# yangsenwxy/VSR

Measured on AMD Instinct MI355X. Metric: voxels/sec fwd+bwd, 4× SR on 16×128×128 cine volumes, 1/2/4/8 MI355X, higher is better.
Workload: dtype bf16

## Files before the change

### vsr_amd/csrc/conv_wgrad_row.hip

```cpp
#include <algorithm>
#include "conv_common.h"

namespace {
using namespace vsrk_conv;

constexpr int RW_NW = 8;
constexpr int RW_KC = 4;
constexpr int RW_SEG = 32 * RW_KC;
constexpr int RW_XV = RW_SEG + 8;
constexpr int RW_XP = RW_XV / 8;
constexpr int RW_YP = RW_SEG / 8;
constexpr int RW_NP = RW_XP + RW_YP;
constexpr int RW_NQ = (RW_NP + RW_NW - 1) / RW_NW;
constexpr int RW_XSLOT = RW_XP * 1024;
constexpr int RW_YSLOT = RW_YP * 1024;
constexpr int RW_NXS = 4, RW_NYS = 2;
constexpr int RW_YBASE = RW_NXS * RW_XSLOT;
constexpr int RW_LDS = RW_YBASE + RW_NYS * RW_YSLOT;
constexpr int RW_COW = 64;
constexpr int RW_SLAB = 9 * RW_COW * 64 + RW_COW;
constexpr uint32_t RW_OOB = 0x80000000u;

#ifndef RW_ABL
#define RW_ABL 0
#endif

__host__ __device__ constexpr int rw_swz(int j) { return 2 * ((j >> 1) & 1) + 4 * ((j >> 3) & 1); }

typedef __amdgpu_buffer_rsrc_t RwRsrc;
__device__ __forceinline__ RwRsrc rw_rsrc(const void* base) {
  const uint64_t b = (uint64_t)base;
  const uint64_t u = ((uint64_t)(uint32_t)__builtin_amdgcn_readfirstlane((int)(uint32_t)(b >> 32)) << 32) |
                     (uint32_t)__builtin_amdgcn_readfirstlane((int)(uint32_t)b);
  return __builtin_amdgcn_make_buffer_rsrc((void*)u, 0, 0x7FFFFFF0, 0x00020000);
}
typedef uint32_t rw_u32x4 __attribute__((ext_vector_type(4)));
__device__ __forceinline__ void rw_st16(uint32_t addr, uint4 v) {
  *(__attribute__((address_space(3))) rw_u32x4*)(size_t)addr = __builtin_bit_cast(rw_u32x4, v);
}

typedef float f32x4_t __attribute__((ext_vector_type(4)));
template <typename H> struct V8R;
template <> struct V8R<bf16> { typedef bf16x8 type; };
template <> struct V8R<f16> { typedef f16x8 type; };
__device__ __forceinline__ f32x4_t rw_mfma(bf16x8 a, bf16x8 b, f32x4_t c) {
  return __builtin_amdgcn_mfma_f32_16x16x32_bf16(a, b, c, 0, 0, 0);
}
__device__ __forceinline__ f32x4_t rw_mfma(f16x8 a, f16x8 b, f32x4_t c) {
  return __builtin_amdgcn_mfma_f32_16x16x32_f16(a, b, c, 0, 0, 0);
}
__device__ __forceinline__ uint4 rw_frag(uint32_t p0, uint32_t p1) {
  const v4i16 a = __builtin_amdgcn_ds_read_tr16_b64_v4i16((lds_v4i16*)(size_t)p0);
  const v4i16 b = __builtin_amdgcn_ds_read_tr16_b64_v4i16((lds_v4i16*)(size_t)p1);
  return __builtin_bit_cast(uint4, __builtin_shufflevector(a, b, 0, 1, 2, 3, 4, 5, 6, 7));
}

constexpr int RW_MAXB = 16;

struct RowArgs {
  const char* x;
  const char* dy;
  int xoff[RW_MAXB], yoff[RW_MAXB];
  uint16_t tapm[RW_MAXB];
  int tapm_x;
  float* ws;
  int64_t xsn, xsd, xsh, xsw, ysn, ysd, ysh, ysw;
  int xd, H, W;
  int bands, band_h, nseg, ncot, ncic, nsplit;
  int want_bias;
  int prio;
};

template <typename H, bool SPM>
__global__ __launch_bounds__(RW_NW * 64, 1) void wgrad_row_kernel(RowArgs a) {
  using V8 = typename V8R<H>::type;
  extern __shared__ __attribute__((aligned(16))) char lds[];
  const int lane = threadIdx.x & 63;
  const int wave = __builtin_amdgcn_readfirstlane(threadIdx.x >> 6);
  const int coh = wave & 1, cib = wave >> 1;

  const int ncombo = a.ncot * a.ncic;
  const int L = xcd_remap(blockIdx.x, a.nsplit * ncombo);
  const int split = L / ncombo;
  const int combo = L - split * ncombo;
  const int cot = combo % a.ncot, cic = combo / a.ncot;
  const int seg = split % a.nseg;
  const int t0 = split / a.nseg;
  const int band = t0 % a.bands, img = t0 / a.bands;
  const int nb = img / a.xd, dd = img - nb * a.xd;
  const int h0 = band * a.band_h;
  const int nst = min(a.H, h0 + a.band_h) - h0;
  const int w0 = seg * RW_SEG;
  const unsigned tapm = SPM ? (unsigned)a.tapm[a.tapm_x ? cic : cot] : 0x1ffu;
  const char* xim = a.x + 2 * (nb * a.xsn + dd * a.xsd + a.xoff[cic]);
  const char* yim = a.dy + 2 * (nb * a.ysn + dd * a.ysd + a.yoff[cot]);

  static_assert(RW_XP == 2 * RW_NW + 1 && RW_YP == 2 * RW_NW, "piece roles");
  uint32_t goff[RW_NQ], loff[RW_NQ];
#pragma unroll
  for (int q = 0; q < RW_NQ; ++q) {
    const bool isx = q != 2 && q != 3;
    const int j = q == 4 ? 2 * RW_NW : wave + RW_NW * (q & 1);
    if (isx) {
      const int v = 8 * j + (lane >> 3);
      const int col = w0 - 1 + v;
      const bool ok = v < RW_SEG + 2 && col >= 0 && col < a.W;
      goff[q] = ok ? (uint32_t)(2 * (col * (int)a.xsw + 8 * (lane & 7))) : RW_OOB;
      loff[q] = (uint32_t)(j * 1024 + (lane >> 3) * 128 + 16 * ((lane & 7) ^ rw_swz(v)));
    } else {
      const int v = 8 * j + (lane >> 3);
      const int col = w0 + v;
      goff[q] = col < a.W ? (uint32_t)(2 * (col * (int)a.ysw + 8 * (lane & 7))) : RW_OOB;
      loff[q] = (uint32_t)(j * 1024 + (lane >> 3) * 128 + 16 * ((lane & 7) ^ rw_swz(v)));
    }
  }
  const uint32_t lbase = lds_addr(lds);
  auto load_set = [&](int t, uint4 (&r)[RW_NQ]) __attribute__((always_inline)) {
    const int xr = h0 - 1 + t;
    const bool xok = xr >= 0 && xr < a.H;
    const int yr = t - 2;
    const bool yok = yr >= 0 && yr < nst;
    const RwRsrc rx = rw_rsrc(xim + 2 * (int64_t)(xok ? xr : 0) * a.xsh);
    const RwRsrc ry = rw_rsrc(yim + 2 * (int64_t)(h0 + (yok ? yr : 0)) * a.ysh);
#pragma unroll
    for (int q = 0; q < RW_NQ; ++q) {
      const bool isx = q != 2 && q != 3;
      if (q == 4 && wave != 0) break;
      r[q] = __builtin_bit_cast(uint4, __builtin_amdgcn_raw_buffer_load_b128(
                                           isx ? rx : ry, (int)((isx ? xok : yok) ? goff[q] : RW_OOB), 0, 0));
    }
  };
  auto store_set = [&](int t, const uint4 (&r)[RW_NQ]) __attribute__((always_inline)) {
    const uint32_t xs = lbase + (uint32_t)(t % RW_NXS) * RW_XSLOT;
    const int yr = t - 2;
    const uint32_t ys = lbase + RW_YBASE + (uint32_t)((yr < 0 ? 0 : yr) % RW_NYS) * RW_YSLOT;
#pragma unroll
    for (int q = 0; q < RW_NQ; ++q) {
      const bool isx = q != 2 && q != 3;
      if (q == 4 && wave != 0) break;
      if (isx) rw_st16(xs + loff[q], r[q]);
      else if (yr >= 0) rw_st16(ys + loff[q], r[q]);
    }
  };

  const int g = lane >> 4, qq = (lane >> 2) & 3, pp = lane & 3;
  uint32_t xo[3][2];
#pragma unroll
  for (int kw = 0; kw < 3; ++kw)
#pragma unroll
    for (int h = 0; h < 2; ++h) {
      const int v = kw + 8 * g + qq + 4 * h;
      xo[kw][h] = (uint32_t)(v * 128 + 16 * ((2 * cib + (pp >> 1)) ^ rw_swz(v)) + 8 * (pp & 1));
    }
  uint32_t yo[2][2];
#pragma unroll
  for (int b = 0; b < 2; ++b)
#pragma unroll
    for (int h = 0; h < 2; ++h) {
      const int v = 8 * g + qq + 4 * h;
      yo[b][h] = (uint32_t)(v * 128 + 16 * ((2 * (2 * coh + b) + (pp >> 1)) ^ rw_swz(v)) + 8 * (pp & 1));
    }

  f32x4_t acc[3][3][2];
#pragma unroll
  for (int i = 0; i < 18; ++i) acc[i / 6][(i / 2) % 3][i % 2] = f32x4_t{0.f, 0.f, 0.f, 0.f};
  f32x4_t bacc[2] = {f32x4_t{0.f, 0.f, 0.f, 0.f}, f32x4_t{0.f, 0.f, 0.f, 0.f}};
  uint4 ones;
  {
    const H one = from_f32<H>(1.f);
    const uint16_t u = __builtin_bit_cast(uint16_t, one);
    const uint32_t w2 = (uint32_t)u | ((uint32_t)u << 16);
    ones = make_uint4(w2, w2, w2, w2);
  }

  const int last = nst + 1;
  uint4 stg[RW_NQ], stg2[RW_NQ];
  load_set(0, stg);
  if (1 <= last) load_set(1, stg2);
  store_set(0, stg);
  if (1 <= last) store_set(1, stg2);
  if (2 <= last) {
    load_set(2, stg);
    store_set(2, stg);
  }
  __syncthreads();
  if (3 <= last) load_set(3, stg);
  __builtin_amdgcn_sched_barrier(0);

  for (int s = 0; s < nst; ++s) {
    uint32_t xa[3][3][2], ya[2][2];
#pragma unroll
    for (int kh = 0; kh < 3; ++kh) {
      const uint32_t xrow = lbase + (uint32_t)((s + kh) % RW_NXS) * RW_XSLOT;
#pragma unroll
      for (int kw = 0; kw < 3; ++kw)
#pragma unroll
        for (int h = 0; h < 2; ++h) {
          xa[kh][kw][h] = xrow + xo[kw][h];
          asm volatile("" : "+v"(xa[kh][kw][h]));
        }
    }
    {
      const uint32_t yr = lbase + RW_YBASE + (uint32_t)(s % RW_NYS) * RW_YSLOT;
#pragma unroll
      for (int b = 0; b < 2; ++b)
#pragma unroll
        for (int h = 0; h < 2; ++h) {
          ya[b][h] = yr + yo[b][h];
          asm volatile("" : "+v"(ya[b][h]));
        }
    }
    uint4 xf[2][3], yf[2][2];
    auto load_group = [&](int G) __attribute__((always_inline)) {
      const int kc = G / 3, kh = G % 3;
      if (kh == 0) {
#pragma unroll
        for (int b = 0; b < 2; ++b) yf[kc & 1][b] = rw_frag(ya[b][0] + kc * 4096, ya[b][1] + kc * 4096);
      }
#pragma unroll
      for (int kw = 0; kw < 3; ++kw) xf[G & 1][kw] = rw_frag(xa[kh][kw][0] + kc * 4096, xa[kh][kw][1] + kc * 4096);
    };
    load_group(0);
#pragma unroll
    for (int G = 0; G < 3 * RW_KC; ++G) {
      if (G + 1 < 3 * RW_KC) load_group(G + 1);
      __builtin_amdgcn_sched_barrier(0);
      if (a.prio) __builtin_amdgcn_s_setprio(1);
      const int kc = G / 3, kh = G % 3;
#pragma unroll
      for (int kw = 0; kw < 3; ++kw) {
        if (SPM && !((tapm >> (kh * 3 + kw)) & 1)) continue;
#pragma unroll
        for (int b = 0; b < 2; ++b)
          if (RW_ABL & 2) acc[kh][kw][b][0] += __builtin_bit_cast(float, yf[kc & 1][b].x ^ xf[G & 1][kw].y);
          else acc[kh][kw][b] = rw_mfma(__builtin_bit_cast(V8, yf[kc & 1][b]), __builtin_bit_cast(V8, xf[G & 1][kw]),
                                   acc[kh][kw][b]);
      }
      if (kh == 1 && kc == cib) {
#pragma unroll
        for (int b = 0; b < 2; ++b)
          bacc[b] = rw_mfma(__builtin_bit_cast(V8, yf[kc & 1][b]), __builtin_bit_cast(V8, ones), bacc[b]);
      }
      if (a.prio) __builtin_amdgcn_s_setprio(0);
      __builtin_amdgcn_sched_barrier(0);
    }
    if (!(RW_ABL & 1)) {
      if (s + 3 <= last) store_set(s + 3, stg);
      asm volatile("s_waitcnt lgkmcnt(0)\n\ts_barrier" ::: "memory");
      if (s + 4 <= last) load_set(s + 4, stg);
    }
    __builtin_amdgcn_sched_barrier(0);
  }

  float* out = a.ws + ((int64_t)split * ncombo + combo) * RW_SLAB;
  const int l15 = lane & 15, lg = lane >> 4;
#pragma unroll
  for (int t9 = 0; t9 < 9; ++t9)
#pragma unroll
    for (int b = 0; b < 2; ++b)
#pragma unroll
      for (int i = 0; i < 4; ++i) {
        const int co = 32 * coh + 16 * b + 4 * lg + i, ci = 16 * cib + l15;
        out[(t9 * RW_COW + co) * 64 + ci] = ((tapm >> t9) & 1) ? acc[t9 / 3][t9 % 3][b][i] : 0.f;
      }
  if (a.want_bias && cic == 0) {
    float* part = reinterpret_cast<float*>(lds);
    __syncthreads();
    if (l15 == 0) {
#pragma unroll
      for (int b = 0; b < 2; ++b)
#pragma unroll
        for (int i = 0; i < 4; ++i) part[cib * 64 + 32 * coh + 16 * b + 4 * lg + i] = bacc[b][i];
    }
    __syncthreads();
    if (threadIdx.x < RW_COW) {
      const int c = threadIdx.x;
      out[9 * RW_COW * 64 + c] = ((part[c] + part[64 + c]) + part[128 + c]) + part[192 + c];
    }
  }
}

const int g_wrow_bands = std::max(0, vsrk_env_int("VSRK_WGRAD_ROW_BANDS", 0));
const int g_wrow_prio = vsrk_env_int("VSRK_WGRAD_ROW_PRIO", 0) == 1;

}

bool vsrk_wgrad_row_plan(const vsrk_conv_desc* d, const vsrk_tensor5* x, const vsrk_tensor5* dy, VsrkRowPlan* p) {
  const int mode = vsrk_path_mode(VSRK_PATH_WGRAD_ROW);
  if (mode == 0) return false;
  if (!vsrk_is16(x->dtype) || dy->dtype != x->dtype) return false;
  if (d->kd != 1 || d->kh != 3 || d->kw != 3 || d->pd != 0 || d->ph != 1 || d->pw != 1) return false;
  if (d->prologue != VSRK_PRO_NONE) return false;
  if (x->c % 64 || dy->c % 64 || (x->shuffle > 1 && dy->shuffle > 1)) return false;
  if (d->subpixel && (x->shuffle > 1 || dy->shuffle > 1) && mode != 2) return false;
  if (x->c / 64 > RW_MAXB || dy->c / 64 > RW_MAXB) return false;
  for (const vsrk_tensor5* t : {x, dy}) {
    if (t->shuffle <= 1) continue;
    const int r = t->shuffle, cph = t->c / (r * r);
    if (cph * r * r != t->c || cph % 64) return false;
  }
  if (x->n != dy->n || x->d != dy->d || x->h != dy->h || x->w != dy->w) return false;
  if (!chunk_ok(x, 2) || !chunk_ok(dy, 2)) return false;
  for (const vsrk_tensor5* t : {x, dy}) {
    const int64_t r = t->shuffle > 1 ? t->shuffle : 1;
    if (t->sn < 0 || t->sd < 0 || t->sh < 0 || t->sw < 0 ||
        (int64_t)(RW_XV + 2) * r * t->sw + (r - 1) * t->sh + t->c >= (1ll << 29))
      return false;
  }
  const int64_t images = (int64_t)x->n * x->d;
  if (images <= 0 || x->h <= 0 || x->w <= 0) return false;
  const int nseg = ceil_div(x->w, RW_SEG);
  const int ncot = dy->c / RW_COW, ncic = x->c / 64;
  const int64_t per_band = images * nseg * ncot * ncic;
  int64_t want = std::max<int64_t>(1, vsrk_num_cus());
  if (vsrk_g_grid_cap > 0) want = std::min<int64_t>(want, vsrk_g_grid_cap);
  int bands = (int)std::max<int64_t>(1, std::min<int64_t>((want + per_band / 2) / per_band, ceil_div(x->h, 8)));
  if (g_wrow_bands > 0) bands = std::min(g_wrow_bands, x->h);
  if (vsrk_g_grid_cap > 0) bands = std::max(1, std::min(bands, x->h));
  p->band_h = ceil_div(x->h, bands);
  p->bands = ceil_div(x->h, p->band_h);
  p->nseg = nseg;
  p->ncot = ncot;
  p->ncic = ncic;
  const int64_t ns = images * p->bands * nseg;
  if (ns * ncot * ncic >= (1ll << 30)) return false;
  p->nsplit = (int)ns;
  p->cot_w = RW_COW;
  p->slab = RW_SLAB;
  p->ws_bytes = (size_t)ns * ncot * ncic * RW_SLAB * sizeof(float);
  return true;
}

int vsrk_conv_wgrad_row(const vsrk_conv_desc* d, const vsrk_tensor5* x, const vsrk_tensor5* dy, int want_bias,
                        float* ws, size_t ws_bytes, VsrkRowPlan* plan, hipStream_t s) {
  VsrkRowPlan p;
  if (!vsrk_wgrad_row_plan(d, x, dy, &p)) return 0;
  if (ws_bytes < p.ws_bytes) return 0;
  RowArgs a;
  a.x = (const char*)x->ptr;
  a.dy = (const char*)dy->ptr;
  a.ws = ws;
  auto blocks = [](const vsrk_tensor5* t, int64_t& sh, int64_t& sw, int* off) {
    const int r = t->shuffle > 1 ? t->shuffle : 1;
    sh = (int64_t)r * t->sh;
    sw = (int64_t)r * t->sw;
    const int cph = t->c / (r * r);
    for (int b = 0; b < t->c / 64; ++b) {
      const int c = 64 * b, sub = c / cph, cc = c - sub * cph;
      off[b] = (int)((sub / r) * t->sh + (sub % r) * t->sw + cc);
    }
  };
  a.xsn = x->sn; a.xsd = x->sd;
  a.ysn = dy->sn; a.ysd = dy->sd;
  blocks(x, a.xsh, a.xsw, a.xoff);
  blocks(dy, a.ysh, a.ysw, a.yoff);
  const vsrk_tensor5* spt = x->shuffle > 1 ? x : (dy->shuffle > 1 ? dy : nullptr);
  const bool spm = d->subpixel && spt;
  a.tapm_x = spt == x;
  if (spm) {
    const int r = spt->shuffle, cph = spt->c / (r * r);
    const int32_t code = d->subpixel & ~(1 << 25);
    for (int b = 0; b < spt->c / 64; ++b) a.tapm[b] = (uint16_t)subpixel_tapmask(code, r, 64 * b / cph);
  }
  a.xd = x->d;
  a.H = x->h;
  a.W = x->w;
  a.bands = p.bands;
  a.band_h = p.band_h;
  a.nseg = p.nseg;
  a.ncot = p.ncot;
  a.ncic = p.ncic;
  a.nsplit = p.nsplit;
  a.want_bias = want_bias;
  a.prio = g_wrow_prio;
  const int grid = p.nsplit * p.ncot * p.ncic;
  vsrk_dispatch16(x->dtype, [&](auto tag) {
    using H = decltype(tag);
    auto kern = spm ? wgrad_row_kernel<H, true> : wgrad_row_kernel<H, false>;
    (void)hipFuncSetAttribute((const void*)kern, hipFuncAttributeMaxDynamicSharedMemorySize, RW_LDS);
    kern<<<grid, RW_NW * 64, RW_LDS, s>>>(a);
    return 0;
  });
  *plan = p;
  return 1;
}
```

Before: 65.30 million.

## Repartition wgrad-row waves across K-chunk halves with LDS cross-wave reduction

Changes the work split in the row weight-gradient kernel. Each wave now owns one 16-wide input-channel block and all 64 output channels, and the two wave groups split the 4 K-chunks two each, instead of splitting output channels in halves. Each x fragment then feeds 4 MFMAs instead of 2, which cuts the LDS read traffic per MFMA. The cost is that the two K halves must be summed through LDS in an epilogue, and accumulator registers double to 36 f32x4. The main loop is also unrolled by the ring depth so slot offsets become immediates, and the unused priority knob is removed.

```diff
diff --git a/vsr_amd/csrc/conv_wgrad_row.hip b/vsr_amd/csrc/conv_wgrad_row.hip
--- a/vsr_amd/csrc/conv_wgrad_row.hip
+++ b/vsr_amd/csrc/conv_wgrad_row.hip
@@ -68,7 +68,6 @@
   int xd, H, W;
   int bands, band_h, nseg, ncot, ncic, nsplit;
   int want_bias;
-  int prio;
 };
 
 template <typename H, bool SPM>
@@ -77,7 +76,7 @@
   extern __shared__ __attribute__((aligned(16))) char lds[];
   const int lane = threadIdx.x & 63;
   const int wave = __builtin_amdgcn_readfirstlane(threadIdx.x >> 6);
-  const int coh = wave & 1, cib = wave >> 1;
+  const int cib = wave & 3, kh2 = wave >> 2;
 
   const int ncombo = a.ncot * a.ncic;
   const int L = xcd_remap(blockIdx.x, a.nsplit * ncombo);
@@ -144,26 +143,45 @@
   };
 
   const int g = lane >> 4, qq = (lane >> 2) & 3, pp = lane & 3;
+  const uint32_t kbase = lbase + (uint32_t)kh2 * (2 * 4096);
   uint32_t xo[3][2];
 #pragma unroll
   for (int kw = 0; kw < 3; ++kw)
 #pragma unroll
     for (int h = 0; h < 2; ++h) {
       const int v = kw + 8 * g + qq + 4 * h;
-      xo[kw][h] = (uint32_t)(v * 128 + 16 * ((2 * cib + (pp >> 1)) ^ rw_swz(v)) + 8 * (pp & 1));
-    }
-  uint32_t yo[2][2];
-#pragma unroll
-  for (int b = 0; b < 2; ++b)
+      xo[kw][h] = kbase + (uint32_t)(v * 128 + 16 * ((2 * cib + (pp >> 1)) ^ rw_swz(v)) + 8 * (pp & 1));
+      asm volatile("" : "+v"(xo[kw][h]));
+    }
+  uint32_t yo[4][2];
+#pragma unroll
+  for (int b = 0; b < 4; ++b)
 #pragma unroll
     for (int h = 0; h < 2; ++h) {
       const int v = 8 * g + qq + 4 * h;
-      yo[b][h] = (uint32_t)(v * 128 + 16 * ((2 * (2 * coh + b) + (pp >> 1)) ^ rw_swz(v)) + 8 * (pp & 1));
-    }
-
-  f32x4_t acc[3][3][2];
-#pragma unroll
-  for (int i = 0; i < 18; ++i) acc[i / 6][(i / 2) % 3][i % 2] = f32x4_t{0.f, 0.f, 0.f, 0.f};
+      yo[b][h] = kbase + RW_YBASE + (uint32_t)(v * 128 + 16 * ((2 * b + (pp >> 1)) ^ rw_swz(v)) + 8 * (pp & 1));
+      asm volatile("" : "+v"(yo[b][h]));
+    }
+  static_assert((RW_NXS - 1) * RW_XSLOT + 4096 < 65536 && (RW_NYS - 1) * RW_YSLOT + 4096 < 65536, "ds offsets");
+
+  const int last = nst + 1;
+  uint4 stg[RW_NQ];
+  {
+    uint4 stg1[RW_NQ], stg2[RW_NQ];
+    load_set(0, stg);
+    load_set(1, stg1);
+    load_set(2, stg2);
+    store_set(0, stg);
+    store_set(1, stg1);
+    store_set(2, stg2);
+  }
+  __syncthreads();
+  if (3 <= last) load_set(3, stg);
+  __builtin_amdgcn_sched_barrier(0);
+
+  f32x4_t acc[3][3][4];
+#pragma unroll
+  for (int i = 0; i < 36; ++i) acc[i / 12][(i / 4) % 3][i % 4] = f32x4_t{0.f, 0.f, 0.f, 0.f};
   f32x4_t bacc[2] = {f32x4_t{0.f, 0.f, 0.f, 0.f}, f32x4_t{0.f, 0.f, 0.f, 0.f}};
   uint4 ones;
   {
@@ -173,115 +191,103 @@
     ones = make_uint4(w2, w2, w2, w2);
   }
 
-  const int last = nst + 1;
-  uint4 stg[RW_NQ], stg2[RW_NQ];
-  load_set(0, stg);
-  if (1 <= last) load_set(1, stg2);
-  store_set(0, stg);
-  if (1 <= last) store_set(1, stg2);
-  if (2 <= last) {
-    load_set(2, stg);
-    store_set(2, stg);
-  }
-  __syncthreads();
-  if (3 <= last) load_set(3, stg);
-  __builtin_amdgcn_sched_barrier(0);
-
-  for (int s = 0; s < nst; ++s) {
-    uint32_t xa[3][3][2], ya[2][2];
-#pragma unroll
-    for (int kh = 0; kh < 3; ++kh) {
-      const uint32_t xrow = lbase + (uint32_t)((s + kh) % RW_NXS) * RW_XSLOT;
-#pragma unroll
-      for (int kw = 0; kw < 3; ++kw)
-#pragma unroll
-        for (int h = 0; h < 2; ++h) {
-          xa[kh][kw][h] = xrow + xo[kw][h];
-          asm volatile("" : "+v"(xa[kh][kw][h]));
+  for (int s4 = 0; s4 < nst; s4 += RW_NXS) {
+#pragma unroll
+    for (int u = 0; u < RW_NXS; ++u) {
+      const int s = s4 + u;
+      if (s >= nst) break;
+      uint4 xf[2][3], yf[4];
+      auto load_x = [&](int G) __attribute__((always_inline)) {
+        const int imm = ((u + G % 3) % RW_NXS) * RW_XSLOT + (G / 3) * 4096;
+#pragma unroll
+        for (int kw = 0; kw < 3; ++kw) xf[G & 1][kw] = rw_frag(xo[kw][0] + imm, xo[kw][1] + imm);
+      };
+      auto load_y = [&](int kc, int b) __attribute__((always_inline)) {
+        const int imm = (u % RW_NYS) * RW_YSLOT + kc * 4096;
+        yf[b] = rw_frag(yo[b][0] + imm, yo[b][1] + imm);
+      };
+#pragma unroll
+      for (int b = 0; b < 4; ++b) load_y(0, b);
+      load_x(0);
+#pragma unroll
+      for (int G = 0; G < 6; ++G) {
+        if (G + 1 < 6) load_x(G + 1);
+        __builtin_amdgcn_sched_barrier(0);
+        const int kc = G / 3, kh = G % 3;
+#pragma unroll
+        for (int b = 0; b < 4; ++b) {
+#pragma unroll
+          for (int kw = 0; kw < 3; ++kw) {
+            if (SPM && !((tapm >> (kh * 3 + kw)) & 1)) continue;
+            if (RW_ABL & 2) acc[kh][kw][b][0] += __builtin_bit_cast(float, yf[b].x ^ xf[G & 1][kw].y);
+            else acc[kh][kw][b] = rw_mfma(__builtin_bit_cast(V8, yf[b]), __builtin_bit_cast(V8, xf[G & 1][kw]),
+                                     acc[kh][kw][b]);
+          }
+          if (kh == 1 && b == cib)
+            bacc[kc] = rw_mfma(__builtin_bit_cast(V8, yf[b]), __builtin_bit_cast(V8, ones), bacc[kc]);
+          if (G == 2) {
+            __builtin_amdgcn_sched_barrier(0);
+            load_y(1, b);
+            __builtin_amdgcn_sched_barrier(0);
+          }
         }
-    }
-    {
-      const uint32_t yr = lbase + RW_YBASE + (uint32_t)(s % RW_NYS) * RW_YSLOT;
-#pragma unroll
-      for (int b = 0; b < 2; ++b)
-#pragma unroll
-        for (int h = 0; h < 2; ++h) {
-          ya[b][h] = yr + yo[b][h];
-          asm volatile("" : "+v"(ya[b][h]));
-        }
-    }
-    uint4 xf[2][3], yf[2][2];
-    auto load_group = [&](int G) __attribute__((always_inline)) {
-      const int kc = G / 3, kh = G % 3;
-      if (kh == 0) {
-#pragma unroll
-        for (int b = 0; b < 2; ++b) yf[kc & 1][b] = rw_frag(ya[b][0] + kc * 4096, ya[b][1] + kc * 4096);
+        __builtin_amdgcn_sched_barrier(0);
       }
-#pragma unroll
-      for (int kw = 0; kw < 3; ++kw) xf[G & 1][kw] = rw_frag(xa[kh][kw][0] + kc * 4096, xa[kh][kw][1] + kc * 4096);
-    };
-    load_group(0);
-#pragma unroll
-    for (int G = 0; G < 3 * RW_KC; ++G) {
-      if (G + 1 < 3 * RW_KC) load_group(G + 1);
+      if (!(RW_ABL & 1)) {
+        if (s + 3 <= last) store_set(s + 3, stg);
+        asm volatile("s_waitcnt lgkmcnt(0)\n\ts_barrier" ::: "memory");
+        if (s + 4 <= last) load_set(s + 4, stg);
+      }
       __builtin_amdgcn_sched_barrier(0);
-      if (a.prio) __builtin_amdgcn_s_setprio(1);
-      const int kc = G / 3, kh = G % 3;
-#pragma unroll
-      for (int kw = 0; kw < 3; ++kw) {
-        if (SPM && !((tapm >> (kh * 3 + kw)) & 1)) continue;
-#pragma unroll
-        for (int b = 0; b < 2; ++b)
-          if (RW_ABL & 2) acc[kh][kw][b][0] += __builtin_bit_cast(float, yf[kc & 1][b].x ^ xf[G & 1][kw].y);
-          else acc[kh][kw][b] = rw_mfma(__builtin_bit_cast(V8, yf[kc & 1][b]), __builtin_bit_cast(V8, xf[G & 1][kw]),
-                                   acc[kh][kw][b]);
-      }
-      if (kh == 1 && kc == cib) {
-#pragma unroll
-        for (int b = 0; b < 2; ++b)
-          bacc[b] = rw_mfma(__builtin_bit_cast(V8, yf[kc & 1][b]), __builtin_bit_cast(V8, ones), bacc[b]);
-      }
-      if (a.prio) __builtin_amdgcn_s_setprio(0);
-      __builtin_amdgcn_sched_barrier(0);
-    }
-    if (!(RW_ABL & 1)) {
-      if (s + 3 <= last) store_set(s + 3, stg);
-      asm volatile("s_waitcnt lgkmcnt(0)\n\ts_barrier" ::: "memory");
-      if (s + 4 <= last) load_set(s + 4, stg);
-    }
-    __builtin_amdgcn_sched_barrier(0);
+    }
   }
 
   float* out = a.ws + ((int64_t)split * ncombo + combo) * RW_SLAB;
   const int l15 = lane & 15, lg = lane >> 4;
-#pragma unroll
-  for (int t9 = 0; t9 < 9; ++t9)
-#pragma unroll
-    for (int b = 0; b < 2; ++b)
-#pragma unroll
-      for (int i = 0; i < 4; ++i) {
-        const int co = 32 * coh + 16 * b + 4 * lg + i, ci = 16 * cib + l15;
-        out[(t9 * RW_COW + co) * 64 + ci] = ((tapm >> t9) & 1) ? acc[t9 / 3][t9 % 3][b][i] : 0.f;
+  constexpr int RW_CMB = 4 * 18 * 1024;
+  static_assert(RW_CMB + 4 * RW_COW * (int)sizeof(float) <= RW_LDS, "combine area");
+  const uint32_t cmb = lbase + (uint32_t)(cib * 18 * 1024 + lane * 16);
+  const bool bias = a.want_bias && cic == 0;
+  float* part = reinterpret_cast<float*>(lds + RW_CMB);
+  __syncthreads();
+  if (bias && l15 == 0) {
+#pragma unroll
+    for (int k = 0; k < 2; ++k)
+#pragma unroll
+      for (int i = 0; i < 4; ++i) part[(2 * kh2 + k) * 64 + 16 * cib + 4 * lg + i] = bacc[k][i];
+  }
+#pragma unroll
+  for (int pass = 0; pass < 2; ++pass) {
+    const bool give = (kh2 == 1) != (pass == 1);
+    if (give) {
+#pragma unroll
+      for (int j = 0; j < 18; ++j) {
+        const int t9 = (18 * pass + j) / 4, b = (18 * pass + j) % 4;
+        *(__attribute__((address_space(3))) f32x4_t*)(size_t)(cmb + j * 1024) = acc[t9 / 3][t9 % 3][b];
       }
-  if (a.want_bias && cic == 0) {
-    float* part = reinterpret_cast<float*>(lds);
+    }
     __syncthreads();
-    if (l15 == 0) {
-#pragma unroll
-      for (int b = 0; b < 2; ++b)
-#pragma unroll
-        for (int i = 0; i < 4; ++i) part[cib * 64 + 32 * coh + 16 * b + 4 * lg + i] = bacc[b][i];
-    }
-    __syncthreads();
-    if (threadIdx.x < RW_COW) {
-      const int c = threadIdx.x;
-      out[9 * RW_COW * 64 + c] = ((part[c] + part[64 + c]) + part[128 + c]) + part[192 + c];
-    }
+    if (!give) {
+#pragma unroll
+      for (int j = 0; j < 18; ++j) {
+        const int t9 = (18 * pass + j) / 4, b = (18 * pass + j) % 4;
+        const f32x4_t o = *(__attribute__((address_space(3))) f32x4_t*)(size_t)(cmb + j * 1024);
+        const f32x4_t v = acc[t9 / 3][t9 % 3][b] + o;
+#pragma unroll
+        for (int i = 0; i < 4; ++i) {
+          const int co = 16 * b + 4 * lg + i, ci = 16 * cib + l15;
+          out[(t9 * RW_COW + co) * 64 + ci] = ((tapm >> t9) & 1) ? v[i] : 0.f;
+        }
+      }
+    }
+  }
+  if (bias && threadIdx.x < RW_COW) {
+    const int c = threadIdx.x;
+    out[9 * RW_COW * 64 + c] = ((part[c] + part[64 + c]) + part[128 + c]) + part[192 + c];
   }
 }
 
 const int g_wrow_bands = std::max(0, vsrk_env_int("VSRK_WGRAD_ROW_BANDS", 0));
-const int g_wrow_prio = vsrk_env_int("VSRK_WGRAD_ROW_PRIO", 0) == 1;
 
 }
 
@@ -372,7 +378,6 @@
   a.ncic = p.ncic;
   a.nsplit = p.nsplit;
   a.want_bias = want_bias;
-  a.prio = g_wrow_prio;
   const int grid = p.nsplit * p.ncot * p.ncic;
   vsrk_dispatch16(x->dtype, [&](auto tag) {
     using H = decltype(tag);
```

Result: faster. 66.04 million, median of 6 (+1.1%).
